# netease-youdao/EmotiVoice

Hardware: NVIDIA H100
Metric: mel_frames_per_sec (higher is better)
Workload: dtype fp32 (fp32 storage + accumulate; tensor-core fp32 emulation: 3xTF32 prefix, bf16x3 after it)

## Files before the change

### emotivoice_b200/csrc/conv1d_gp.cu

```cuda
#include "ev_common.cuh"
#include "gp_pipeline.cuh"

namespace ev {
namespace gp {

using namespace gpl;

constexpr int MAX_A = 8;

struct GPlan {
  int BN, mt, kbg, planes;
  int rows_pad;
  int a_plane_bytes, b_plane_bytes, a_stage_bytes, b_stage_bytes;
  int a_stages, b_stages;
  int acc_cols;
  int tiles_m, tiles_n, total_tiles;
  int smem_total;
};

__host__ __device__ inline bool make_gplan(const GpConvParams& p, int mode, int BN, int mt, int kbg, GPlan* o, int span = -1, int kmin = 0, int ng = 1) {
  if (span < 0) span = (p.K - 1) * p.dil;
  if (kmin <= 0) kmin = p.K;
  GPlan q;
  q.planes = mode == 1 ? 2 : 1;
  const int b_planes = (mode == 1 || mode == 3) ? 2 : 1;
  const int cpg = mode == 2 ? 8 : 4;
  const int wcpg = mode >= 2 ? 8 : 4;
  q.kbg = kbg; q.mt = mt; q.BN = BN;
  if (mt * BN > 2 * ACC_REGS) return false;
  q.acc_cols = mt * BN;
  const int rows = BM * mt + span;
  q.rows_pad = (rows + 7) / 8 * 8;
  q.a_plane_bytes = kbg * q.rows_pad * 16;
  q.b_plane_bytes = (kbg * cpg / wcpg) * BN * 16;
  q.a_stage_bytes = q.planes * q.a_plane_bytes;
  q.b_stage_bytes = b_planes * q.b_plane_bytes;
  const int budget = 227 * 1024 - SMEM_HEAD;
  const int n_cb = (p.Cin + cpg * kbg - 1) / (cpg * kbg);
  const int b_max = n_cb * kmin < MAX_B ? n_cb * kmin : MAX_B;
  if (!grow_stages(q.a_stage_bytes, q.b_stage_bytes, budget, MAX_A, b_max, &q.a_stages, &q.b_stages)) return false;
  q.tiles_m = (p.L + BM * mt - 1) / (BM * mt);
  q.tiles_n = (p.Cout + BN - 1) / BN;
  q.total_tiles = ng * p.B * q.tiles_m * q.tiles_n;
  q.smem_total = SMEM_HEAD + q.a_stages * q.a_stage_bytes + q.b_stages * q.b_stage_bytes;
  *o = q;
  return true;
}

template <int MODE, int MT, int KBG, int BN>
__global__ void __launch_bounds__(THREADS, 1) conv1d_gp_kernel(const __grid_constant__ GpConvParams p, const __grid_constant__ GPlan pl,
                                                               const __grid_constant__ GpGroups gs) {
  constexpr bool BF16 = (MODE == 2);
  constexpr bool X3B = (MODE == 3);
  constexpr bool OP16 = BF16 || X3B;
  constexpr int CPG = BF16 ? 8 : 4;
  constexpr int WCPG = OP16 ? 8 : 4;
  constexpr int KB = CPG * KBG;
  constexpr int NA = ACC_REGS / MT;
  constexpr int NK8 = KB / (2 * WCPG);
  static_assert(!X3B || KBG % 4 == 0, "bf16x3 consumes four fp32 granules (16 channels) per MMA K step");
  static_assert(MT * BN <= 2 * ACC_REGS, "accumulators of the tile exceed the register budget");
  extern __shared__ __align__(128) uint8_t smem_raw[];
  const int tid = threadIdx.x;
  const int warp = __shfl_sync(0xffffffffu, tid >> 5, 0);
  const int lane = tid & 31;

  uint8_t* a_tiles = smem_raw + SMEM_HEAD;
  uint8_t* b_tiles = a_tiles + pl.a_stages * pl.a_stage_bytes;
  const Ring<MAX_A> ring{smem_u32(smem_raw)};
  if (tid == 0) ring.init(pl.a_stages, pl.b_stages);
  __syncthreads();

  asm volatile("griddepcontrol.launch_dependents;" ::: "memory");

  const int n_cb = (p.Cin + KB - 1) / KB;
  const int tiles_per_b = pl.tiles_m * pl.tiles_n;
  const int tiles_per_g = p.B * tiles_per_b;

  auto decode = [&](int tile, int& gi, int& b, int& t0, int& n0, int& len) {
    gi = tile / tiles_per_g;
    tile -= gi * tiles_per_g;
    b = tile / tiles_per_b;
    const int r = tile - b * tiles_per_b;
    const int tm = r / pl.tiles_n, tn = r - tm * pl.tiles_n;
    t0 = tm * (BM * MT);
    n0 = tn * BN;
    len = p.lens ? min(p.L, p.lens[b] * p.lens_mul) : p.L;
  };

  if (warp < NCW) {
    asm volatile("griddepcontrol.wait;" ::: "memory");
    const int wg = warp >> 2, wl = warp & 3;
    const int coutR = p.Cout / p.rate;
    const int gout = coutR / CPG;
    const size_t Lout = (size_t)p.L * p.rate;
    const int accm = p.acc;
    const uint32_t a_lbo = (uint32_t)pl.rows_pad * 16u, b_lbo = (uint32_t)BN * 16u;
    const uint64_t a_desc0 = make_desc(0u, X3B ? 2u * a_lbo : a_lbo, 128u), b_desc0 = make_desc(0u, b_lbo, 128u);
    const uint32_t a_k8 = (X3B ? 4u : 2u) * a_lbo;
    const uint32_t a_lo_off = X3B ? a_lbo : (uint32_t)pl.a_plane_bytes;
    float acc[MT][NA];
#pragma unroll
    for (int mt = 0; mt < MT; ++mt)
#pragma unroll
      for (int i = 0; i < NA; ++i) acc[mt][i] = 0.f;
    int a_cnt = 0, b_cnt = 0;
    for (int tile = blockIdx.x; tile < pl.total_tiles; tile += gridDim.x) {
      int gi, b, t0, n0, len;
      decode(tile, gi, b, t0, n0, len);
      if (t0 >= len) continue;
      const GpGroup& G = gs.g[gi];
      const int K = G.K;
      const uint32_t a_tap = (uint32_t)G.dil * 16u;
      OneBehind<MAX_A> rel{ring, lane};
      for (int cb = 0; cb < n_cb; ++cb, ++a_cnt) {
        const int sa = a_cnt % pl.a_stages;
        const int nk8 = min(KB, p.Cin - cb * KB) / (2 * WCPG);
        mbar_wait(ring.a_ready(sa), (a_cnt / pl.a_stages) & 1);
        const uint64_t a_hi0 = desc_advance(a_desc0, smem_u32(a_tiles + sa * pl.a_stage_bytes) + (uint32_t)(wg * 64) * 16u);
        for (int j = 0; j < K; ++j, ++b_cnt) {
          const int sb = b_cnt % pl.b_stages;
          mbar_wait(ring.b_full(sb), (b_cnt / pl.b_stages) & 1);
          const uint64_t b_hi0 = desc_advance(b_desc0, smem_u32(b_tiles + sb * pl.b_stage_bytes));
          const uint64_t a_j = desc_advance(a_hi0, (uint32_t)j * a_tap);
          if (nk8 == NK8) {
            tap_chain<MODE, BN, NK8>(acc, a_j, a_k8, a_lo_off, b_hi0, (uint32_t)pl.b_plane_bytes, cb | j);
            wgmma_wait<1>();
          } else {
            tap_chain_short<MODE, BN>(acc, a_j, a_k8, a_lo_off, b_hi0, (uint32_t)pl.b_plane_bytes, cb | j, nk8);
            wgmma_wait<1>();
          }
          rel.step(sb, j == K - 1 ? sa : -1);
        }
      }

      constexpr int EQ = MT == 1 ? 2 : 1;
      const bool has_res = G.res != nullptr;
      const int row0 = t0 + wg * 64 + frag_row(0, lane, wl);
      float2 ebias[EQ];
      pair_t<BF16> eres[EQ][MT][2], eout[EQ][MT][2];
      auto column = [&](int q, int& n) {
        n = n0 + frag_col(4 * q, lane);
// ... 31 lines not shown
            for (int h = 0; h < 2; ++h) {
              const int row = row0 + mt * BM + 8 * h;
              if (row >= len) continue;
              const int i = 4 * (ch * EQ + q) + 2 * h;
              float v0 = acc[mt][i], v1 = acc[mt][i + 1];
              if (G.bias) { v0 += ebias[q].x; v1 += ebias[q].y; }
              if (has_res) {
                const float2 r = unpack_pair(eres[q][mt][h]);
                v0 += r.x; v1 += r.y;
              }
              if (accm != EV_ACC_STORE) {
                const float2 o = unpack_pair(eout[q][mt][h]);
                v0 += o.x; v1 += o.y;
                if (accm == EV_ACC_ADD_DIV) { v0 /= p.div; v1 /= p.div; }
              }
              store_pair<BF16>(G.out, ec + (size_t)row * p.rate * CPG, v0, v1);
            }
        }
      };
      epi_load(0);
      wgmma_wait<0>();
      rel.drain();
#pragma unroll
      for (int ch = 0; ch < NA / 4 / EQ; ++ch) {
        if (ch > 0) epi_load(ch);
        epi_store(ch);
      }
    }
  } else if (warp < W_ALOAD) {
    const int xt = (warp - W_XFORM) * 32 + lane;
    int a_cnt = 0;
    for (int tile = blockIdx.x; tile < pl.total_tiles; tile += gridDim.x) {
      int gi, b, t0, n0, len;
      decode(tile, gi, b, t0, n0, len);
      if (t0 >= len) continue;
      const int span = (gs.g[gi].K - 1) * gs.g[gi].dil;
      transform_tile<MODE, KBG>(ring, a_cnt, pl.a_stages, a_tiles, pl.a_stage_bytes, pl.a_plane_bytes, pl.rows_pad, p.Cin, t0 - span / 2,
                                           BM * MT + span, len, p.in_act == EV_ACT_LRELU, p.in_slope, xt);
    }
  } else if (warp == W_ALOAD) {
    if (lane == 0) {
      asm volatile("griddepcontrol.wait;" ::: "memory");
      int a_cnt = 0;
      for (int tile = blockIdx.x; tile < pl.total_tiles; tile += gridDim.x) {
        int gi, b, t0, n0, len;
        decode(tile, gi, b, t0, n0, len);
        if (t0 >= len) continue;
        const int span = (gs.g[gi].K - 1) * gs.g[gi].dil;
        load_x_tile<CPG, KBG>(ring, a_cnt, pl.a_stages, a_tiles, pl.a_stage_bytes, pl.rows_pad, gs.g[gi].x, b, p.Cin, p.L, t0 - span / 2,
                              BM * MT + span, len);
      }
    }
    __syncwarp();
  } else {
    if (lane == 0) {
      const int bnp = p.Cout < 128 ? p.Cout : 128;
      const int win = p.Cin / WCPG;
      int b_cnt = 0;
      for (int tile = blockIdx.x; tile < pl.total_tiles; tile += gridDim.x) {
        int gi, b, t0, n0, len;
        decode(tile, gi, b, t0, n0, len);
        if (t0 >= len) continue;
        const int K = gs.g[gi].K;
        const size_t tile_stride = (size_t)K * win * bnp * 4;
        const float* wt = gs.g[gi].w + (size_t)(n0 / bnp) * tile_stride + (size_t)(n0 % bnp) * 4;
        load_w_tile<MODE, KBG, BN>(ring, b_cnt, pl.b_stages, b_tiles, pl.b_stage_bytes, pl.b_plane_bytes, wt, K, p.Cin, p.Cout, bnp);
      }
    }
    __syncwarp();
  }
}

template <bool BF16>
__global__ void __launch_bounds__(256) to_gp_kernel(const float* __restrict__ in, long long sb, long long st_, long long sc, void* __restrict__ out,
                                                    int B, int L, int C) {
  asm volatile("griddepcontrol.launch_dependents;\n\tgriddepcontrol.wait;" ::: "memory");
  constexpr int CPG = BF16 ? 8 : 4;
  const int G = C / CPG;
  const size_t i = (size_t)blockIdx.x * blockDim.x + threadIdx.x;
  if (i >= (size_t)B * G * L) return;
  const int t = (int)(i % L);
  const int g = (int)((i / L) % G);
  const int b = (int)(i / ((size_t)L * G));
  const float* src = in + (size_t)b * sb + (size_t)t * st_ + (size_t)(g * CPG) * sc;
  float v[CPG];
#pragma unroll
  for (int e = 0; e < CPG; ++e) v[e] = src[(size_t)e * sc];
  uint4 o;
  if (BF16) {
    o.x = pack_bf16(v[0], v[1]); o.y = pack_bf16(v[2], v[3]); o.z = pack_bf16(v[CPG - 4], v[CPG - 3]); o.w = pack_bf16(v[CPG - 2], v[CPG - 1]);
  } else {
    o.x = __float_as_uint(v[0]); o.y = __float_as_uint(v[1]); o.z = __float_as_uint(v[2]); o.w = __float_as_uint(v[3]);
  }
  reinterpret_cast<uint4*>(out)[i] = o;
}

template <int N>
__global__ void __launch_bounds__(256) gp_sum_div_kernel(const float4* __restrict__ a, const float4* __restrict__ b, const float4* __restrict__ c,
                                                         float4* __restrict__ out, size_t n4, float div) {
  asm volatile("griddepcontrol.launch_dependents;\n\tgriddepcontrol.wait;" ::: "memory");
  const size_t i = (size_t)blockIdx.x * blockDim.x + threadIdx.x;
  if (i >= n4) return;
  const float4 va = a[i], vb = b[i];
  float4 t = make_float4(vb.x + va.x, vb.y + va.y, vb.z + va.z, vb.w + va.w);
  if (N == 3) {
    const float4 vc = c[i];
    t = make_float4(vc.x + t.x, vc.y + t.y, vc.z + t.z, vc.w + t.w);
// ... 88 lines not shown
#pragma unroll
    for (int e = 0; e < CPG; ++e) xs[(size_t)(g * CPG + e) * RS + r] = lrelu_f(f[e], slope);
  }
  for (int i = threadIdx.x; i < C * KP; i += GP4_T) {
    const int c = i / KP, j = i - c * KP;
    ws[i] = j < K ? w[j * C + c] : 0.f;
  }
  __syncthreads();
  float acc[GP4_O];
#pragma unroll
  for (int o = 0; o < GP4_O; ++o) acc[o] = 0.f;
  for (int c = 0; c < C; ++c) {
    float xw[NW * 4], wv[KP];
    const float4* xr = reinterpret_cast<const float4*>(xs + (size_t)c * RS + GP4_O * threadIdx.x);
    const float4* wr = reinterpret_cast<const float4*>(ws + c * KP);
#pragma unroll
    for (int q = 0; q < NW; ++q) { const float4 v = xr[q]; xw[4 * q] = v.x; xw[4 * q + 1] = v.y; xw[4 * q + 2] = v.z; xw[4 * q + 3] = v.w; }
#pragma unroll
    for (int q = 0; q < KP / 4; ++q) { const float4 v = wr[q]; wv[4 * q] = v.x; wv[4 * q + 1] = v.y; wv[4 * q + 2] = v.z; wv[4 * q + 3] = v.w; }
#pragma unroll
    for (int j = 0; j < K; ++j)
#pragma unroll
      for (int o = 0; o < GP4_O; ++o) acc[o] = fmaf(xw[o + j], wv[j], acc[o]);
  }
  const float b0 = bias[0];
  float r[GP4_O];
#pragma unroll
  for (int o = 0; o < GP4_O; ++o) r[o] = t + o < len ? tanhf(acc[o] + b0) : 0.f;
  if (vec) *reinterpret_cast<float4*>(out) = make_float4(r[0], r[1], r[2], r[3]);
  else for (int o = 0; o < GP4_O; ++o) if (t + o < L) out[o] = r[o];
}

}

static int validate_gp(const GpConvParams& p, int mode) {
  EV_CHECK_ARG(p.B > 0 && p.L > 0, "conv1d_gp: bad problem B=%d L=%d", p.B, p.L);
  EV_CHECK_ARG(mode >= 0 && mode <= 3, "conv1d_gp: mode %d", mode);
  EV_CHECK_ARG(p.Cin % (mode >= 2 ? 16 : 8) == 0, "conv1d_gp: Cin=%d must be a multiple of %d", p.Cin, mode >= 2 ? 16 : 8);
  EV_CHECK_ARG(p.Cout % 32 == 0 && (p.Cout <= 128 || p.Cout % 128 == 0), "conv1d_gp: Cout=%d must be a multiple of 32, and of 128 above 128", p.Cout);
  EV_CHECK_ARG(p.rate >= 1 && p.Cout % p.rate == 0 && (p.Cout / p.rate) % 32 == 0, "conv1d_gp: rate=%d does not split Cout=%d into multiples of 32", p.rate, p.Cout);
  EV_CHECK_ARG(p.K >= 1 && (p.K & 1) && p.dil >= 1, "conv1d_gp: K=%d must be odd, dil=%d >= 1", p.K, p.dil);
  EV_CHECK_ARG(p.in_act == EV_ACT_NONE || p.in_act == EV_ACT_LRELU, "conv1d_gp: unsupported input activation");
  EV_CHECK_ARG(p.rate == 1 || (!p.res && p.acc == EV_ACC_STORE), "conv1d_gp: residual / accumulate need rate == 1");
  EV_CHECK_ARG((long long)p.L * p.rate < (1ll << 31), "conv1d_gp: output too long");
  return EV_OK;
}

int gp_shape_kbg(const GpConvParams& p, int mode) {
  gp::GPlan pl;
  const int bn_max = p.Cout <= 128 ? p.Cout : 128;
  return (mode != 1 && gp::make_gplan(p, mode, bn_max, 1, 8, &pl)) ? 8 : 4;
}

static int plan_gp(const GpConvParams& p, int mode, gp::GPlan* out, int ng = 1, int ksum = 0, int span = -1, int kmin = 0, int kbg_forced = 0,
                   const int* gK = nullptr) {
  EV_TRY(validate_gp(p, mode));
  const int nsm = sm_count();
  const int kbg = kbg_forced ? kbg_forced : gp_shape_kbg(p, mode);
  if (ksum <= 0) ksum = p.K;
  if (span < 0) span = (p.K - 1) * p.dil;
  const double kc8 = (double)ksum / ng * p.Cin / 8.0;
  const double n_mma = ((mode == 1 || mode == 3) ? 3.0 : 1.0) * (mode >= 2 ? 0.5 : 1.0) * kc8;
  const double w_per_n = ((mode == 1 || mode == 3) ? 2.0 : 1.0) * (mode >= 2 ? 16.0 : 32.0) / 42.0;
  const double esize = mode == 2 ? 2.0 : 4.0;
  double best = 1e300;
  bool found = false;
  gp::GPlan best_pl;
  const int bn_max = p.Cout <= 128 ? p.Cout : 128;
  for (int BN = bn_max; BN >= bn_max; BN /= 2) {
    if (p.Cout % BN || BN % 32) continue;
    for (int mt = 4; mt >= 1; mt >>= 1) {
      gp::GPlan pl;
      if (!gp::make_gplan(p, mode, BN, mt, kbg, &pl, span, kmin, ng)) continue;
      double c_mma = BN / 2.0;
      if (32.0 + BN / 4.0 > c_mma) c_mma = 32.0 + BN / 4.0;
      const double t_mma = mt * n_mma * c_mma;
      const double t_w = w_per_n * BN * kc8;
      const double t_hbm = (double)mt * tc::BM * ((double)p.Cin * (mt * tc::BM + span) / (mt * tc::BM) + 2.0 * BN) * esize / 23.0;
      double t = t_mma > t_w ? t_mma : t_w;
      if (t_hbm > t) t = t_hbm;
      double cost;
      if (ng > 1 && gK) {
        const int tg = pl.total_tiles / ng;
        const int ncta = pl.total_tiles < nsm ? pl.total_tiles : nsm;
        cost = 0.0;
        for (int c = 0; c < ncta; ++c) {
          double sum = 0.0;
          for (int i = c; i < pl.total_tiles; i += nsm) sum += t * gK[i / tg] * ng / (double)ksum + 3000.0;
          if (sum > cost) cost = sum;
        }
      } else {
        const double waves = (double)((pl.total_tiles + nsm - 1) / nsm);
        cost = waves * (t + 3000.0);
      }
      if (cost < best * 0.97) { best = cost; best_pl = pl; found = true; }
    }
  }
  if (!found) { set_error("conv1d_gp: tile does not fit in shared memory / accumulator registers (K=%d dil=%d Cout=%d)", p.K, p.dil, p.Cout); return EV_EINVAL; }
  *out = best_pl;
  return EV_OK;
}

int gp_solo_tiles(const GpConvParams& p, int mode) {
  gp::GPlan pl;
  return plan_gp(p, mode, &pl) == EV_OK ? pl.total_tiles : 0;
}

int debug_gp_plan(const GpConvParams& p, int mode, int* v) {
  gp::GPlan pl;
  const int rc = plan_gp(p, mode, &pl);
  if (rc != EV_OK) return rc;
  v[0] = pl.BN; v[1] = pl.mt; v[2] = pl.kbg; v[3] = pl.a_stages; v[4] = pl.b_stages; v[5] = gp::NTW;
  v[6] = pl.planes; v[7] = pl.acc_cols; v[8] = pl.smem_total; v[9] = pl.total_tiles; v[10] = pl.rows_pad;
  return EV_OK;
}

using GpKernel = void (*)(GpConvParams, gp::GPlan, GpGroups);
template <int MODE, int KBG>
static GpKernel gp_kernel_tile(int mt, int bn) {
  switch (bn) {
    case 128: return mt == 1 ? gp::conv1d_gp_kernel<MODE, 1, KBG, 128> : nullptr;
    case 96: return mt == 1 ? gp::conv1d_gp_kernel<MODE, 1, KBG, 96> : nullptr;
    case 64: return mt == 2 ? gp::conv1d_gp_kernel<MODE, 2, KBG, 64> : mt == 1 ? gp::conv1d_gp_kernel<MODE, 1, KBG, 64> : nullptr;
    case 32: return mt == 4 ? gp::conv1d_gp_kernel<MODE, 4, KBG, 32> : mt == 2 ? gp::conv1d_gp_kernel<MODE, 2, KBG, 32>
                  : mt == 1 ? gp::conv1d_gp_kernel<MODE, 1, KBG, 32> : nullptr;
    default: return nullptr;
  }
}
static GpKernel gp_kernel(int mode, int kbg, int mt, int bn) {
  if (mode == 1) return kbg == 4 ? gp_kernel_tile<1, 4>(mt, bn) : nullptr;
  if (mode == 3) return kbg == 8 ? gp_kernel_tile<3, 8>(mt, bn) : gp_kernel_tile<3, 4>(mt, bn);
  if (mode == 2) return kbg == 8 ? gp_kernel_tile<2, 8>(mt, bn) : gp_kernel_tile<2, 4>(mt, bn);
  return kbg == 8 ? gp_kernel_tile<0, 8>(mt, bn) : gp_kernel_tile<0, 4>(mt, bn);
}

static int dispatch_gp(const GpConvParams& p, const gp::GPlan& pl, const GpGroups& gs, int mode, cudaStream_t st) {
  static std::atomic<uint64_t> attr_devs{0};
  if (first_use_on_device(attr_devs)) preload_conv1d_gp();
  const GpKernel k = gp_kernel(mode, pl.kbg, pl.mt, pl.BN);
  EV_CHECK_ARG(k, "conv1d_gp: no kernel for mode %d, KBG %d, MT %d, BN %d", mode, pl.kbg, pl.mt, pl.BN);
  const int nsm = sm_count();
  const int grid = pl.total_tiles < nsm ? pl.total_tiles : nsm;
  return launch("conv1d_gp_kernel", k, (unsigned)grid, gpl::THREADS, pl.smem_total, st, p, pl, gs);
}

int launch_conv1d_gp(const GpConvParams& p, int mode, cudaStream_t st) {
  gp::GPlan pl;
  EV_TRY(plan_gp(p, mode, &pl));
  GpGroups gs{};
  gs.ng = 1;
  gs.g[0] = GpGroup{p.x, p.w, p.bias, p.res, p.out, p.K, p.dil};
  return dispatch_gp(p, pl, gs, mode, st);
}

static bool group_shapes_match(const GpConvParams* ps, int n, int mode, int* kbg) {
  if (n < 1 || n > 3) return false;
  const GpConvParams& a = ps[0];
  int kb = 0;
  for (int i = 0; i < n; ++i) {
    const GpConvParams& q = ps[i];
    if (q.B != a.B || q.L != a.L || q.Cin != a.Cin || q.Cout != a.Cout || q.rate != 1 || q.lens != a.lens || q.lens_mul != a.lens_mul ||
        q.in_act != a.in_act || q.in_slope != a.in_slope || q.acc != EV_ACC_STORE || !q.x || !q.w || !q.out)
      return false;
    if (q.K < 1 || !(q.K & 1) || q.dil < 1) return false;
    for (int j = 0; j < i; ++j)
      if (ps[j].out == q.out) return false;
    const int k = gp_shape_kbg(q, mode);
    if (i == 0) kb = k;
    else if (k != kb) return false;
  }
  *kbg = kb;
  return true;
}
bool gp_group_supported(const GpConvParams* ps, int n, int mode) {
  int kbg = 0;
  if (mode < 0 || mode > 3 || !group_shapes_match(ps, n, mode, &kbg)) return false;
  return validate_gp(ps[0], mode) == EV_OK;
}
static int plan_group(const GpConvParams* ps, int n, int mode, GpGroups* gs_out, gp::GPlan* pl_out);
int debug_gp_group_plan(const GpConvParams* ps, int n, int mode, int* v) {
  GpGroups gs{};
  gp::GPlan pl;
  EV_TRY(plan_group(ps, n, mode, &gs, &pl));
  v[0] = pl.BN; v[1] = pl.mt; v[2] = pl.kbg; v[3] = pl.a_stages; v[4] = pl.b_stages; v[5] = gp::NTW;
  v[6] = pl.planes; v[7] = pl.acc_cols; v[8] = pl.smem_total; v[9] = pl.total_tiles; v[10] = pl.rows_pad;
  return EV_OK;
}
int launch_conv1d_gp_group(const GpConvParams* ps, int n, int mode, cudaStream_t st) {
  GpGroups gs{};
  gp::GPlan pl;
  EV_TRY(plan_group(ps, n, mode, &gs, &pl));
  return dispatch_gp(ps[0], pl, gs, mode, st);
}
static int plan_group(const GpConvParams* ps, int n, int mode, GpGroups* gs_out, gp::GPlan* pl_out) {
  GpGroups& gs = *gs_out;
  gp::GPlan& pl = *pl_out;
  int kbg = 0;
  EV_CHECK_ARG(ps && group_shapes_match(ps, n, mode, &kbg), "conv1d_gp group: the %d convolutions do not share a launch shape", n);
  int order[3];
  gpl::heaviest_first(ps, n, order);
  gs = GpGroups{};
  gs.ng = n;
  int ksum = 0, span = 0, kmin = 1 << 30;
  for (int i = 0; i < n; ++i) {
    const GpConvParams& q = ps[order[i]];
    gs.g[i] = GpGroup{q.x, q.w, q.bias, q.res, q.out, q.K, q.dil};
    ksum += q.K;
    span = (q.K - 1) * q.dil > span ? (q.K - 1) * q.dil : span;
    kmin = q.K < kmin ? q.K : kmin;
  }
  int gK[3] = {0, 0, 0};
  for (int i = 0; i < n; ++i) gK[i] = gs.g[i].K;
  return plan_gp(ps[0], mode, &pl, n, ksum, span, kmin, kbg, gK);
}

void preload_conv1d_gp() {
  for (int mode = 0; mode < 4; ++mode)
    for (int kbg = 4; kbg <= 8; kbg += 4)
      for (int bn = 32; bn <= 128; bn += 32)
        for (int mt = 1; mt * bn <= 128; mt *= 2)
          if (const GpKernel k = gp_kernel(mode, kbg, mt, bn)) cudaFuncSetAttribute(k, cudaFuncAttributeMaxDynamicSharedMemorySize, 227 * 1024);
  cudaFuncSetAttribute(gp::conv_post_gp_kernel<false>, cudaFuncAttributeMaxDynamicSharedMemorySize, 160 * 1024);
  cudaFuncSetAttribute(gp::conv_post_gp_kernel<true>, cudaFuncAttributeMaxDynamicSharedMemorySize, 160 * 1024);
  cudaFuncSetAttribute(gp::conv_post_gp4_kernel<false, 7>, cudaFuncAttributeMaxDynamicSharedMemorySize, 112 * 1024);
  cudaFuncSetAttribute(gp::conv_post_gp4_kernel<true, 7>, cudaFuncAttributeMaxDynamicSharedMemorySize, 112 * 1024);
  cudaFuncAttributes fa;
  cudaFuncGetAttributes(&fa, gp::to_gp_kernel<false>);
  cudaFuncGetAttributes(&fa, gp::to_gp_kernel<true>);
  cudaGetLastError();
}

int launch_to_gp(const float* in, long long sb, long long st_, long long sc, void* out, int B, int L, int C, int bf16, cudaStream_t st) {
  EV_CHECK_ARG(B > 0 && L > 0 && C % (bf16 ? 8 : 4) == 0, "to_gp: B=%d L=%d C=%d", B, L, C);
  const size_t n = (size_t)B * (C / (bf16 ? 8 : 4)) * L;
  const unsigned grid = (unsigned)((n + 255) / 256);
  return launch("to_gp_kernel", bf16 ? gp::to_gp_kernel<true> : gp::to_gp_kernel<false>, grid, 256, 0, st, in, sb, st_, sc, out, B, L, C);
}

int launch_gp_sum_div(const float* a, const float* b, const float* c, float* out, size_t n_floats, float div, cudaStream_t st) {
  EV_CHECK_ARG(a && b && out && n_floats % 4 == 0, "gp_sum_div: bad arguments");
  const size_t n4 = n_floats / 4;
  const unsigned grid = (unsigned)((n4 + 255) / 256);
  const float4 *a4 = reinterpret_cast<const float4*>(a), *b4 = reinterpret_cast<const float4*>(b), *c4 = reinterpret_cast<const float4*>(c);
  float4* o4 = reinterpret_cast<float4*>(out);
  return launch("gp_sum_div_kernel", c ? gp::gp_sum_div_kernel<3> : gp::gp_sum_div_kernel<2>, grid, 256, 0, st, a4, b4, c4, o4, n4, div);
}

int launch_conv_post_gp(const void* x, int bf16, const float* w, const float* bias, const int32_t* lens, int lens_mul, int B, int L, int C, int K,
                        float slope, float* wav, cudaStream_t st) {
  EV_CHECK_ARG(C % (bf16 ? 8 : 4) == 0 && C <= 128 && K <= 15 && (K & 1), "conv_post_gp: C=%d K=%d", C, K);
  EV_CHECK_ARG(B > 0 && B <= 65535 && L > 0, "conv_post_gp: bad shape");
  const size_t smem = (size_t)(C * (gp::GPP_BT + K - 1) + K * C) * sizeof(float);
  static std::atomic<uint64_t> attr_devs{0};
  if (first_use_on_device(attr_devs)) {
    cudaFuncSetAttribute(gp::conv_post_gp_kernel<false>, cudaFuncAttributeMaxDynamicSharedMemorySize, 160 * 1024);
    cudaFuncSetAttribute(gp::conv_post_gp_kernel<true>, cudaFuncAttributeMaxDynamicSharedMemorySize, 160 * 1024);
    cudaFuncSetAttribute(gp::conv_post_gp4_kernel<false, 7>, cudaFuncAttributeMaxDynamicSharedMemorySize, 112 * 1024);
    cudaFuncSetAttribute(gp::conv_post_gp4_kernel<true, 7>, cudaFuncAttributeMaxDynamicSharedMemorySize, 112 * 1024);
  }
  if (K == 7 && C <= 48) {
    constexpr int RS = gp::GP4_ROWS + 8;
    const size_t smem4 = (size_t)C * (RS + 8) * sizeof(float);
    dim3 grid4((L + gp::GP4_ROWS - 1) / gp::GP4_ROWS, B);
    return launch("conv_post_gp4_kernel", bf16 ? gp::conv_post_gp4_kernel<true, 7> : gp::conv_post_gp4_kernel<false, 7>, grid4, gp::GP4_T, smem4,
                  st, x, w, bias, lens, lens_mul, L, C, slope, wav);
  }
  dim3 grid((L + gp::GPP_BT - 1) / gp::GPP_BT, B);
  return launch("conv_post_gp_kernel", bf16 ? gp::conv_post_gp_kernel<true> : gp::conv_post_gp_kernel<false>, grid, gp::GPP_BT, smem, st, x, w,
                bias, lens, lens_mul, L, C, K, slope, wav);
}

}
```

### emotivoice_b200/csrc/gp_pipeline.cuh

```cuda
#pragma once
#include "tc_common.cuh"

namespace ev {
namespace gpl {

using namespace tc;

constexpr int NCW = 8;
constexpr int NTW = 4;
constexpr int W_XFORM = NCW;
constexpr int W_ALOAD = W_XFORM + NTW;
constexpr int W_BLOAD = W_ALOAD + 1;
constexpr int THREADS = (W_BLOAD + 1) * 32;
constexpr int MAX_B = 8;
constexpr int SMEM_HEAD = 1024;
constexpr int XF_UNROLL = 4;

__device__ __forceinline__ float lrelu_f(float v, float slope) { return fmaxf(v, v * slope); }

template <int MAX_A>
struct Ring {
  uint32_t base;
  __device__ __forceinline__ uint32_t a_full(int s) const { return base + 8u * s; }
  __device__ __forceinline__ uint32_t a_ready(int s) const { return base + 8u * (MAX_A + s); }
  __device__ __forceinline__ uint32_t a_empty(int s) const { return base + 8u * (2 * MAX_A + s); }
  __device__ __forceinline__ uint32_t b_full(int s) const { return base + 8u * (3 * MAX_A + s); }
  __device__ __forceinline__ uint32_t b_empty(int s) const { return base + 8u * (3 * MAX_A + MAX_B + s); }
  __device__ __forceinline__ void init(int a_stages, int b_stages) const {
    for (int s = 0; s < a_stages; ++s) { mbar_init(a_full(s), 1); mbar_init(a_ready(s), NTW * 32); mbar_init(a_empty(s), NCW); }
    for (int s = 0; s < b_stages; ++s) { mbar_init(b_full(s), 1); mbar_init(b_empty(s), NCW); }
    asm volatile("fence.mbarrier_init.release.cluster;" ::: "memory");
  }
};

__host__ __device__ inline bool grow_stages(int a_bytes, int b_bytes, int budget, int a_max, int b_max, int* a_stages, int* b_stages) {
  auto fits = [&](int a, int b) { return a * a_bytes + b * b_bytes <= budget; };
  int a = 2, b = b_max < 2 ? b_max : 2;
  if (!fits(a, b)) return false;
  while (b < b_max && b < 4 && fits(a, b + 1)) ++b;
  while (a < 4 && fits(a + 1, b)) ++a;
  while (b < b_max && fits(a, b + 1)) ++b;
  while (a < a_max && fits(a + 1, b)) ++a;
  *a_stages = a;
  *b_stages = b;
  return true;
}

template <class P>
inline void heaviest_first(const P* ps, int n, int order[3]) {
  order[0] = 0; order[1] = 1; order[2] = 2;
  for (int i = 0; i < n; ++i)
    for (int j = i + 1; j < n; ++j)
      if (ps[order[j]].K > ps[order[i]].K) { const int t = order[i]; order[i] = order[j]; order[j] = t; }
}

template <int CPG, int KBG, int MAX_A>
__device__ __forceinline__ void load_x_tile(Ring<MAX_A> ring, int& a_cnt, int a_stages, uint8_t* x_tiles, int stage_bytes, int rows_pad,
                                            const void* x, int b, int C, int L, int row0, int rows, int len) {
  constexpr int KB = CPG * KBG;
  const int n_cb = (C + KB - 1) / KB;
  const int r_lo = max(row0, 0);
  const int r_hi = min(row0 + rows, len);
  const uint32_t nbytes = (uint32_t)(r_hi - r_lo) * 16u, roff = (uint32_t)(r_lo - row0) * 16u;
  const uint8_t* xb = reinterpret_cast<const uint8_t*>(x) + ((size_t)b * (C / CPG) * L + r_lo) * 16;
  for (int cb = 0; cb < n_cb; ++cb, ++a_cnt) {
    const int s = a_cnt % a_stages;
    const int ngran = min(KB, C - cb * KB) / CPG;
    mbar_wait(ring.a_empty(s), ((a_cnt / a_stages) & 1) ^ 1);
    mbar_expect_tx(ring.a_full(s), (uint32_t)ngran * nbytes);
// ... 140 lines not shown
```

### emotivoice_b200/csrc/resblock_gp.cu

```cuda
#include "ev_common.cuh"
#include "gp_pipeline.cuh"

namespace ev {
namespace gpp {

using namespace gpl;

constexpr int MAX_A = 6;
constexpr int PAIR_THREADS = 512;
__host__ __device__ constexpr int cons_regs(int acc_cols) { return acc_cols == 2 * ACC_REGS ? 216 : 208; }
__host__ __device__ constexpr int prod_regs(int acc_cols) { return (65536 / 128 - 2 * cons_regs(acc_cols)) / 2; }
template <int N>
__device__ __forceinline__ void setmaxnreg_inc() { asm volatile("setmaxnreg.inc.sync.aligned.u32 %0;" ::"n"(N)); }
template <int N>
__device__ __forceinline__ void setmaxnreg_dec() { asm volatile("setmaxnreg.dec.sync.aligned.u32 %0;" ::"n"(N)); }
template <bool BF16>
__device__ __forceinline__ pair_t<BF16> load_pair_if(bool on, const void* t, size_t e) {
  if constexpr (BF16) {
    uint32_t v = 0u;
    asm volatile("{\n\t.reg .pred p;\n\tsetp.ne.b32 p, %2, 0;\n\t@p ld.global.b32 %0, [%1];\n\t}"
                 : "+r"(v) : "l"(reinterpret_cast<const uint16_t*>(t) + e), "r"((int)on));
    return v;
  } else {
    float2 v = make_float2(0.f, 0.f);
    asm volatile("{\n\t.reg .pred p;\n\tsetp.ne.b32 p, %3, 0;\n\t@p ld.global.v2.f32 {%0, %1}, [%2];\n\t}"
                 : "+f"(v.x), "+f"(v.y) : "l"(reinterpret_cast<const float*>(t) + e), "r"((int)on));
    return v;
  }
}
template <bool BF16>
__device__ __forceinline__ void store_pair_if(bool on, void* t, size_t e, float v0, float v1) {
  if constexpr (BF16)
    asm volatile("{\n\t.reg .pred p;\n\tsetp.ne.b32 p, %2, 0;\n\t@p st.global.b32 [%0], %1;\n\t}"
                 :: "l"(reinterpret_cast<uint16_t*>(t) + e), "r"(pack_bf16(v0, v1)), "r"((int)on) : "memory");
  else
    asm volatile("{\n\t.reg .pred p;\n\tsetp.ne.b32 p, %3, 0;\n\t@p st.global.v2.f32 [%0], {%1, %2};\n\t}"
                 :: "l"(reinterpret_cast<float*>(t) + e), "f"(v0), "f"(v1), "r"((int)on) : "memory");
}

struct PPlan {
  int mt, kbg;
  int rows1_pad, rows2_pad, R;
  int x_plane_bytes, x_stage_bytes, a2_plane_bytes, a2_bytes, b_plane_bytes, b_stage_bytes;
  int a_stages, b_stages;
  int acc_cols;
  int tiles_m, total_tiles;
  int smem_total;
};

__host__ __device__ inline bool make_pplan(const GpPairParams& p, int mode, int mt, int kbg, PPlan* o, int span1 = -1, int kmax = 0) {
  if (span1 < 0) span1 = (p.K - 1) * p.dil;
  if (kmax <= 0) kmax = p.K;
  PPlan q;
  q.mt = mt; q.kbg = kbg;
  const int C = p.C;
  if (C > 128 || C % 32 || mt * C > 2 * ACC_REGS) return false;
  const int cpg = mode == 2 ? 8 : 4;
  const int ocpg = mode >= 2 ? 8 : 4;
  const int xplanes = mode == 1 ? 2 : 1;
  const int splitp = (mode == 1 || mode == 3) ? 2 : 1;
  q.R = BM * mt - (p.K - 1);
  if (BM * mt - (kmax - 1) < 32) return false;
  const int rows1 = BM * mt + span1;
  q.rows1_pad = (rows1 + 7) / 8 * 8;
  q.rows2_pad = (BM * mt + (kmax - 1) + 7) / 8 * 8;
  q.x_plane_bytes = kbg * q.rows1_pad * 16;
  q.x_stage_bytes = xplanes * q.x_plane_bytes;
  q.a2_plane_bytes = (C / ocpg) * q.rows2_pad * 16;
  q.a2_bytes = splitp * q.a2_plane_bytes;
  q.b_plane_bytes = (kbg * cpg / ocpg) * C * 16;
  q.b_stage_bytes = splitp * q.b_plane_bytes;
  const int budget = 227 * 1024 - SMEM_HEAD - q.a2_bytes;
  if (!grow_stages(q.x_stage_bytes, q.b_stage_bytes, budget, MAX_A, MAX_B, &q.a_stages, &q.b_stages)) return false;
  q.acc_cols = mt * C;
  q.tiles_m = (p.L + q.R - 1) / q.R;
  q.total_tiles = p.B * q.tiles_m;
  q.smem_total = SMEM_HEAD + q.a2_bytes + q.a_stages * q.x_stage_bytes + q.b_stages * q.b_stage_bytes;
  *o = q;
  return true;
}

template <int MODE, int MT, int KBG, int C>
__global__ void __launch_bounds__(PAIR_THREADS, 1) resblock_gp_kernel(const __grid_constant__ GpPairParams p, const __grid_constant__ PPlan pl,
                                                                     const __grid_constant__ GpPairGroups gs) {
  constexpr bool SPLIT3 = (MODE == 1), BF16 = (MODE == 2), X3B = (MODE == 3);
  constexpr bool OP16 = BF16 || X3B;
  constexpr int CPG = BF16 ? 8 : 4;
  constexpr int OCPG = OP16 ? 8 : 4;
  constexpr int KB = CPG * KBG;
  constexpr int KBGW = KBG * CPG / OCPG;
  constexpr int NA = ACC_REGS / MT;
  constexpr int NQ = C / 8;
  constexpr int NK = (C < KB ? C : KB) / (2 * OCPG);
  static_assert(C % KB == 0 || C < KB, "every channel block has NK K steps");
  static_assert(!X3B || KBG % 4 == 0, "bf16x3 consumes four fp32 granules per MMA K step");
  static_assert(MT * C <= 2 * ACC_REGS, "accumulators of the tile exceed the register budget");
  extern __shared__ __align__(128) uint8_t smem_raw[];
  const int tid = threadIdx.x, lane = tid & 31;
  const int warp = __shfl_sync(0xffffffffu, tid >> 5, 0);

  uint8_t* a2_tile = smem_raw + SMEM_HEAD;
  uint8_t* x_tiles = a2_tile + pl.a2_bytes;
  uint8_t* b_tiles = x_tiles + pl.a_stages * pl.x_stage_bytes;
  const Ring<MAX_A> ring{smem_u32(smem_raw)};
  if (tid == 0) ring.init(pl.a_stages, pl.b_stages);
  __syncthreads();
  asm volatile("griddepcontrol.launch_dependents;" ::: "memory");
  if (warp < NCW) setmaxnreg_inc<cons_regs(MT * C)>();
  else setmaxnreg_dec<prod_regs(MT * C)>();

  const int n_cb = (C + KB - 1) / KB;
  const int gC = C / CPG;
  auto group_of = [&](int tile) { return (gs.ng > 1 && tile >= gs.g[1].tile0) ? ((gs.ng > 2 && tile >= gs.g[2].tile0) ? 2 : 1) : 0; };
  auto tile_len = [&](int tile, int& gi, int& b, int& t0) {
    gi = group_of(tile);
    const int local = tile - gs.g[gi].tile0;
    b = local / gs.g[gi].tiles_m;
    t0 = (local - b * gs.g[gi].tiles_m) * gs.g[gi].R;
    return p.lens ? min(p.L, p.lens[b] * p.lens_mul) : p.L;
  };
  auto active = [&](int tile) { int gi, b, t0; const int len = tile_len(tile, gi, b, t0); return t0 < len; };
  auto next_active = [&](int tile) {
    while (tile < pl.total_tiles && !active(tile)) tile += gridDim.x;
    return tile;
  };

  if (warp < NCW) {
    asm volatile("griddepcontrol.wait;" ::: "memory");
    const int wg = warp >> 2, wl = warp & 3;
    const float slope = p.slope;
    const uint32_t x_lbo = (uint32_t)pl.rows1_pad * 16u, a2_lbo = (uint32_t)pl.rows2_pad * 16u, b_lbo = (uint32_t)C * 16u;
    const uint64_t x_desc0 = make_desc(0u, X3B ? 2u * x_lbo : x_lbo, 128u), b_desc0 = make_desc(0u, b_lbo, 128u);
    const uint64_t a2_desc0 = make_desc(smem_u32(a2_tile) + (uint32_t)(wg * 64) * 16u, a2_lbo, 128u);
    const uint32_t x_k = (X3B ? 4u : 2u) * x_lbo, x_lo_off = X3B ? x_lbo : (uint32_t)pl.x_plane_bytes;
    float acc1[MT][NA], acc2[MT][NA];
#pragma unroll
    for (int mt = 0; mt < MT; ++mt)
#pragma unroll
      for (int i = 0; i < NA; ++i) {
        acc1[mt][i] = 0.f;
        asm volatile("mov.b32 %0, 0;" : "=f"(acc2[mt][i]));
      }
    int a_cnt = 0, b_cnt = 0;
    int e_tile = -1, e_gi = 0, e_b = 0, e_t0 = 0, e_len = 0;
    const int rl0 = wg * 64 + frag_row(0, lane, wl);
    auto epi2_chunk = [&](int q, auto div) {
      const GpPairGroup& E = gs.g[e_gi];
      const int c = frag_col(4 * q, lane);
      const size_t ec = ((size_t)e_b * gC + c / CPG) * p.L * CPG + (c % CPG);
      const float2 ebias = __ldg(reinterpret_cast<const float2*>(E.b2 + c));
      const bool accm = p.acc != EV_ACC_STORE;
      pair_t<BF16> eres[MT][2], eout[MT][2];
#pragma unroll
      for (int mt = 0; mt < MT; ++mt)
#pragma unroll
        for (int h = 0; h < 2; ++h) {
          const int rl = rl0 + mt * BM + 8 * h, row = e_t0 + rl;
          const bool ok = rl < E.R && row < e_len;
          const size_t e = ec + (size_t)row * CPG;
          eres[mt][h] = load_pair_if<BF16>(ok, E.x, e);
          eout[mt][h] = load_pair_if<BF16>(ok && accm, E.out, e);
        }
// ... 178 lines not shown
  const int kbg = pair_shape_kbg(p, mode);
  const int nsm = sm_count();
  for (int mt = 4; mt >= 1; mt >>= 1) {
    gpp::PPlan pl;
    if (!gpp::make_pplan(p, mode, mt, kbg, &pl)) continue;
    if (mt > 1 && pl.total_tiles < nsm) {
      gpp::PPlan smaller;
      if (gpp::make_pplan(p, mode, mt / 2, kbg, &smaller)) continue;
    }
    *out = pl;
    return true;
  }
  return false;
}

bool gp_pair_supported(const GpPairParams& p, int mode) {
  gpp::PPlan pl;
  return plan_pair(p, mode, &pl) && pl.mt >= 2;
}

int debug_gp_pair_plan(const GpPairParams& p, int mode, int* v) {
  gpp::PPlan pl;
  if (!plan_pair(p, mode, &pl)) { set_error("resblock_gp: shape not supported (C=%d K=%d dil=%d mode=%d)", p.C, p.K, p.dil, mode); return EV_EINVAL; }
  v[0] = pl.mt; v[1] = pl.kbg; v[2] = pl.a_stages; v[3] = pl.b_stages; v[4] = gpp::NTW; v[5] = pl.acc_cols; v[6] = pl.smem_total;
  v[7] = pl.total_tiles; v[8] = pl.R; v[9] = pl.rows1_pad; v[10] = pl.rows2_pad;
  return EV_OK;
}

using PairKernel = void (*)(GpPairParams, gpp::PPlan, GpPairGroups);
template <int MODE, int KBG>
static PairKernel pair_kernel_tile(int mt, int c) {
  switch (c) {
    case 128: return mt == 1 ? gpp::resblock_gp_kernel<MODE, 1, KBG, 128> : nullptr;
    case 64: return mt == 2 ? gpp::resblock_gp_kernel<MODE, 2, KBG, 64> : mt == 1 ? gpp::resblock_gp_kernel<MODE, 1, KBG, 64> : nullptr;
    case 32: return mt == 4 ? gpp::resblock_gp_kernel<MODE, 4, KBG, 32> : mt == 2 ? gpp::resblock_gp_kernel<MODE, 2, KBG, 32>
                  : mt == 1 ? gpp::resblock_gp_kernel<MODE, 1, KBG, 32> : nullptr;
    default: return nullptr;
  }
}
static PairKernel pair_kernel(int mode, int kbg, int mt, int c) {
  if (mode == 1) return kbg == 4 ? pair_kernel_tile<1, 4>(mt, c) : nullptr;
  if (mode == 3) return kbg == 8 ? pair_kernel_tile<3, 8>(mt, c) : pair_kernel_tile<3, 4>(mt, c);
  if (mode == 2) return kbg == 8 ? pair_kernel_tile<2, 8>(mt, c) : pair_kernel_tile<2, 4>(mt, c);
  return kbg == 8 ? pair_kernel_tile<0, 8>(mt, c) : pair_kernel_tile<0, 4>(mt, c);
}

static int dispatch_pair(const GpPairParams& p, const gpp::PPlan& pl, const GpPairGroups& gs, int mode, cudaStream_t st) {
  static std::atomic<uint64_t> attr_devs{0};
  if (first_use_on_device(attr_devs)) preload_resblock_gp();
  const PairKernel k = pair_kernel(mode, pl.kbg, pl.mt, p.C);
  EV_CHECK_ARG(k, "resblock_gp: no kernel for mode %d, KBG %d, MT %d, C %d", mode, pl.kbg, pl.mt, p.C);
  const int nsm = sm_count();
  const int grid = pl.total_tiles < nsm ? pl.total_tiles : nsm;
  return launch("resblock_gp_kernel", k, (unsigned)grid, gpp::PAIR_THREADS, pl.smem_total, st, p, pl, gs);
}

void preload_resblock_gp() {
  for (int mode = 0; mode < 4; ++mode)
    for (int kbg = 4; kbg <= 8; kbg += 4)
      for (int c = 32; c <= 128; c *= 2)
        for (int mt = 1; mt * c <= 128; mt *= 2)
          if (const PairKernel k = pair_kernel(mode, kbg, mt, c)) cudaFuncSetAttribute(k, cudaFuncAttributeMaxDynamicSharedMemorySize, 227 * 1024);
  cudaGetLastError();
}

int launch_gp_pair(const GpPairParams& p, int mode, cudaStream_t st) {
  gpp::PPlan pl;
  if (!plan_pair(p, mode, &pl)) { set_error("resblock_gp: shape not supported (C=%d K=%d dil=%d mode=%d)", p.C, p.K, p.dil, mode); return EV_EINVAL; }
  GpPairGroups gs{};
  gs.ng = 1;
  gs.g[0] = GpPairGroup{p.x, p.w1, p.b1, p.w2, p.b2, p.out, p.K, p.dil, pl.R, pl.tiles_m, 0};
  return dispatch_pair(p, pl, gs, mode, st);
}

int gp_pair_solo_tiles(const GpPairParams& p, int mode) {
  gpp::PPlan pl;
  return plan_pair(p, mode, &pl) ? pl.total_tiles : 0;
}

static bool plan_pair_group(const GpPairParams* ps, int n, int mode, GpPairGroups* gs, gpp::PPlan* out) {
  if (!ps || n < 1 || n > 3) return false;
  const GpPairParams& a = ps[0];
  int kbg = 0, span1 = 0, kmax = 0;
  for (int i = 0; i < n; ++i) {
    const GpPairParams& q = ps[i];
    if (q.B != a.B || q.L != a.L || q.C != a.C || q.lens != a.lens || q.lens_mul != a.lens_mul || q.slope != a.slope || q.acc != EV_ACC_STORE) return false;
    if (!q.x || !q.out || !q.w1 || !q.w2 || !q.b1 || !q.b2 || q.x == q.out) return false;
    for (int j = 0; j < n; ++j)
      if (j != i && (ps[j].out == q.out || ps[j].out == q.x)) return false;
    gpp::PPlan solo;
    if (!plan_pair(q, mode, &solo) || solo.mt < 2) return false;
    if (i == 0) kbg = solo.kbg;
    else if (solo.kbg != kbg) return false;
    span1 = (q.K - 1) * q.dil > span1 ? (q.K - 1) * q.dil : span1;
    kmax = q.K > kmax ? q.K : kmax;
  }
  int order[3];
  gpl::heaviest_first(ps, n, order);
  const int nsm = sm_count();
  for (int mt = 4; mt >= 2; mt >>= 1) {
    gpp::PPlan pl;
    if (!gpp::make_pplan(a, mode, mt, kbg, &pl, span1, kmax)) continue;
    int total = 0;
    gs->ng = n;
    for (int i = 0; i < n; ++i) {
      const GpPairParams& q = ps[order[i]];
      const int R = tc::BM * mt - (q.K - 1);
// ... 37 lines not shown
```

Measured before the change: 128,000.

## Allow wide MT=2, BN=128 conv tiles with warp-specialized register rebalancing

```diff
diff --git a/emotivoice_b200/csrc/conv1d_gp.cu b/emotivoice_b200/csrc/conv1d_gp.cu
--- a/emotivoice_b200/csrc/conv1d_gp.cu
+++ b/emotivoice_b200/csrc/conv1d_gp.cu
@@ -1,3 +1,4 @@
+#include <cstdlib>
 #include "ev_common.cuh"
 #include "gp_pipeline.cuh"
 
@@ -7,6 +8,9 @@
 using namespace gpl;
 
 constexpr int MAX_A = 8;
+constexpr int MAX_COLS = 256;
+__host__ __device__ constexpr bool wide_tile(int mt, int bn) { return mt * bn > 2 * ACC_REGS; }
+__host__ __device__ constexpr int kernel_threads(int mt, int bn) { return wide_tile(mt, bn) ? SPLIT_THREADS : THREADS; }
 
 struct GPlan {
   int BN, mt, kbg, planes;
@@ -27,7 +31,7 @@
   const int cpg = mode == 2 ? 8 : 4;
   const int wcpg = mode >= 2 ? 8 : 4;
   q.kbg = kbg; q.mt = mt; q.BN = BN;
-  if (mt * BN > 2 * ACC_REGS) return false;
+  if (mt * BN > MAX_COLS || (wide_tile(mt, BN) && BN != 128)) return false;
   q.acc_cols = mt * BN;
   const int rows = BM * mt + span;
   q.rows_pad = (rows + 7) / 8 * 8;
@@ -48,7 +52,7 @@
 }
 
 template <int MODE, int MT, int KBG, int BN>
-__global__ void __launch_bounds__(THREADS, 1) conv1d_gp_kernel(const __grid_constant__ GpConvParams p, const __grid_constant__ GPlan pl,
+__global__ void __launch_bounds__(kernel_threads(MT, BN), 1) conv1d_gp_kernel(const __grid_constant__ GpConvParams p, const __grid_constant__ GPlan pl,
                                                                const __grid_constant__ GpGroups gs) {
   constexpr bool BF16 = (MODE == 2);
   constexpr bool X3B = (MODE == 3);
@@ -56,10 +60,11 @@
   constexpr int CPG = BF16 ? 8 : 4;
   constexpr int WCPG = OP16 ? 8 : 4;
   constexpr int KB = CPG * KBG;
-  constexpr int NA = ACC_REGS / MT;
+  constexpr bool WIDE = wide_tile(MT, BN);
+  constexpr int NA = WIDE ? BN / 2 : ACC_REGS / MT;
   constexpr int NK8 = KB / (2 * WCPG);
   static_assert(!X3B || KBG % 4 == 0, "bf16x3 consumes four fp32 granules (16 channels) per MMA K step");
-  static_assert(MT * BN <= 2 * ACC_REGS, "accumulators of the tile exceed the register budget");
+  static_assert(MT * BN <= MAX_COLS && (!WIDE || BN == 128), "accumulators of the tile exceed the register budget");
   extern __shared__ __align__(128) uint8_t smem_raw[];
   const int tid = threadIdx.x;
   const int warp = __shfl_sync(0xffffffffu, tid >> 5, 0);
@@ -88,6 +93,7 @@
     len = p.lens ? min(p.L, p.lens[b] * p.lens_mul) : p.L;
   };
 
+  if constexpr (WIDE) split_registers<MT * BN>(warp);
   if (warp < NCW) {
     asm volatile("griddepcontrol.wait;" ::: "memory");
     const int wg = warp >> 2, wl = warp & 3;
@@ -225,7 +231,7 @@
       }
     }
     __syncwarp();
-  } else {
+  } else if (!WIDE || warp == W_BLOAD) {
     if (lane == 0) {
       const int bnp = p.Cout < 128 ? p.Cout : 128;
       const int win = p.Cin / WCPG;
@@ -420,6 +426,13 @@
   return (mode != 1 && gp::make_gplan(p, mode, bn_max, 1, 8, &pl)) ? 8 : 4;
 }
 
+static int gp_max_acc_cols(const GpConvParams& p, int mode, int ng) {
+  if (!(mode == 3 && p.Cin >= 256 && p.rate == 1 && ng == 1)) return 2 * tc::ACC_REGS;
+  const char* e = getenv("EV_GP_MAX_ACC_COLS");
+  const int v = e ? atoi(e) : 0;
+  return v > 0 && v < gp::MAX_COLS ? v : gp::MAX_COLS;
+}
+
 static int plan_gp(const GpConvParams& p, int mode, gp::GPlan* out, int ng = 1, int ksum = 0, int span = -1, int kmin = 0, int kbg_forced = 0,
                    const int* gK = nullptr) {
   EV_TRY(validate_gp(p, mode));
@@ -435,11 +448,12 @@
   bool found = false;
   gp::GPlan best_pl;
   const int bn_max = p.Cout <= 128 ? p.Cout : 128;
+  const int max_cols = gp_max_acc_cols(p, mode, ng);
   for (int BN = bn_max; BN >= bn_max; BN /= 2) {
     if (p.Cout % BN || BN % 32) continue;
     for (int mt = 4; mt >= 1; mt >>= 1) {
       gp::GPlan pl;
-      if (!gp::make_gplan(p, mode, BN, mt, kbg, &pl, span, kmin, ng)) continue;
+      if (mt * BN > max_cols || !gp::make_gplan(p, mode, BN, mt, kbg, &pl, span, kmin, ng)) continue;
       double c_mma = BN / 2.0;
       if (32.0 + BN / 4.0 > c_mma) c_mma = 32.0 + BN / 4.0;
       const double t_mma = mt * n_mma * c_mma;
@@ -487,7 +501,10 @@
 template <int MODE, int KBG>
 static GpKernel gp_kernel_tile(int mt, int bn) {
   switch (bn) {
-    case 128: return mt == 1 ? gp::conv1d_gp_kernel<MODE, 1, KBG, 128> : nullptr;
+    case 128:
+      if constexpr (MODE == 3)
+        if (mt == 2) return gp::conv1d_gp_kernel<MODE, 2, KBG, 128>;
+      return mt == 1 ? gp::conv1d_gp_kernel<MODE, 1, KBG, 128> : nullptr;
     case 96: return mt == 1 ? gp::conv1d_gp_kernel<MODE, 1, KBG, 96> : nullptr;
     case 64: return mt == 2 ? gp::conv1d_gp_kernel<MODE, 2, KBG, 64> : mt == 1 ? gp::conv1d_gp_kernel<MODE, 1, KBG, 64> : nullptr;
     case 32: return mt == 4 ? gp::conv1d_gp_kernel<MODE, 4, KBG, 32> : mt == 2 ? gp::conv1d_gp_kernel<MODE, 2, KBG, 32>
@@ -509,7 +526,7 @@
   EV_CHECK_ARG(k, "conv1d_gp: no kernel for mode %d, KBG %d, MT %d, BN %d", mode, pl.kbg, pl.mt, pl.BN);
   const int nsm = sm_count();
   const int grid = pl.total_tiles < nsm ? pl.total_tiles : nsm;
-  return launch("conv1d_gp_kernel", k, (unsigned)grid, gpl::THREADS, pl.smem_total, st, p, pl, gs);
+  return launch("conv1d_gp_kernel", k, (unsigned)grid, gp::kernel_threads(pl.mt, pl.BN), pl.smem_total, st, p, pl, gs);
 }
 
 int launch_conv1d_gp(const GpConvParams& p, int mode, cudaStream_t st) {
@@ -586,7 +603,7 @@
   for (int mode = 0; mode < 4; ++mode)
     for (int kbg = 4; kbg <= 8; kbg += 4)
       for (int bn = 32; bn <= 128; bn += 32)
-        for (int mt = 1; mt * bn <= 128; mt *= 2)
+        for (int mt = 1; mt * bn <= gp::MAX_COLS; mt *= 2)
           if (const GpKernel k = gp_kernel(mode, kbg, mt, bn)) cudaFuncSetAttribute(k, cudaFuncAttributeMaxDynamicSharedMemorySize, 227 * 1024);
   cudaFuncSetAttribute(gp::conv_post_gp_kernel<false>, cudaFuncAttributeMaxDynamicSharedMemorySize, 160 * 1024);
   cudaFuncSetAttribute(gp::conv_post_gp_kernel<true>, cudaFuncAttributeMaxDynamicSharedMemorySize, 160 * 1024);
diff --git a/emotivoice_b200/csrc/gp_pipeline.cuh b/emotivoice_b200/csrc/gp_pipeline.cuh
--- a/emotivoice_b200/csrc/gp_pipeline.cuh
+++ b/emotivoice_b200/csrc/gp_pipeline.cuh
@@ -15,6 +15,19 @@
 constexpr int MAX_B = 8;
 constexpr int SMEM_HEAD = 1024;
 constexpr int XF_UNROLL = 4;
+
+constexpr int SPLIT_THREADS = 512;
+__host__ __device__ constexpr int cons_regs(int acc_cols) { return acc_cols == 4 * ACC_REGS ? 216 : 208; }
+__host__ __device__ constexpr int prod_regs(int acc_cols) { return (65536 / 128 - 2 * cons_regs(acc_cols)) / 2; }
+template <int N>
+__device__ __forceinline__ void setmaxnreg_inc() { asm volatile("setmaxnreg.inc.sync.aligned.u32 %0;" ::"n"(N)); }
+template <int N>
+__device__ __forceinline__ void setmaxnreg_dec() { asm volatile("setmaxnreg.dec.sync.aligned.u32 %0;" ::"n"(N)); }
+template <int ACC_COLS>
+__device__ __forceinline__ void split_registers(int warp) {
+  if (warp < NCW) setmaxnreg_inc<cons_regs(ACC_COLS)>();
+  else setmaxnreg_dec<prod_regs(ACC_COLS)>();
+}
 
 __device__ __forceinline__ float lrelu_f(float v, float slope) { return fmaxf(v, v * slope); }
 
diff --git a/emotivoice_b200/csrc/resblock_gp.cu b/emotivoice_b200/csrc/resblock_gp.cu
--- a/emotivoice_b200/csrc/resblock_gp.cu
+++ b/emotivoice_b200/csrc/resblock_gp.cu
@@ -7,13 +7,6 @@
 using namespace gpl;
 
 constexpr int MAX_A = 6;
-constexpr int PAIR_THREADS = 512;
-__host__ __device__ constexpr int cons_regs(int acc_cols) { return acc_cols == 2 * ACC_REGS ? 216 : 208; }
-__host__ __device__ constexpr int prod_regs(int acc_cols) { return (65536 / 128 - 2 * cons_regs(acc_cols)) / 2; }
-template <int N>
-__device__ __forceinline__ void setmaxnreg_inc() { asm volatile("setmaxnreg.inc.sync.aligned.u32 %0;" ::"n"(N)); }
-template <int N>
-__device__ __forceinline__ void setmaxnreg_dec() { asm volatile("setmaxnreg.dec.sync.aligned.u32 %0;" ::"n"(N)); }
 template <bool BF16>
 __device__ __forceinline__ pair_t<BF16> load_pair_if(bool on, const void* t, size_t e) {
   if constexpr (BF16) {
@@ -81,7 +74,7 @@
 }
 
 template <int MODE, int MT, int KBG, int C>
-__global__ void __launch_bounds__(PAIR_THREADS, 1) resblock_gp_kernel(const __grid_constant__ GpPairParams p, const __grid_constant__ PPlan pl,
+__global__ void __launch_bounds__(SPLIT_THREADS, 1) resblock_gp_kernel(const __grid_constant__ GpPairParams p, const __grid_constant__ PPlan pl,
                                                                      const __grid_constant__ GpPairGroups gs) {
   constexpr bool SPLIT3 = (MODE == 1), BF16 = (MODE == 2), X3B = (MODE == 3);
   constexpr bool OP16 = BF16 || X3B;
@@ -106,8 +99,7 @@
   if (tid == 0) ring.init(pl.a_stages, pl.b_stages);
   __syncthreads();
   asm volatile("griddepcontrol.launch_dependents;" ::: "memory");
-  if (warp < NCW) setmaxnreg_inc<cons_regs(MT * C)>();
-  else setmaxnreg_dec<prod_regs(MT * C)>();
+  split_registers<2 * MT * C>(warp);
 
   const int n_cb = (C + KB - 1) / KB;
   const int gC = C / CPG;
@@ -392,7 +384,7 @@
   EV_CHECK_ARG(k, "resblock_gp: no kernel for mode %d, KBG %d, MT %d, C %d", mode, pl.kbg, pl.mt, p.C);
   const int nsm = sm_count();
   const int grid = pl.total_tiles < nsm ? pl.total_tiles : nsm;
-  return launch("resblock_gp_kernel", k, (unsigned)grid, gpp::PAIR_THREADS, pl.smem_total, st, p, pl, gs);
+  return launch("resblock_gp_kernel", k, (unsigned)grid, gpp::SPLIT_THREADS, pl.smem_total, st, p, pl, gs);
 }
 
 void preload_resblock_gp() {
```

After: 127,500, median of 6. No clear change (-0.3%).
